# facebookresearch/co-tracker

Measured on AMD Instinct MI355X. Metric: tracked-point-frames/sec (N*T/s), higher is better.
Workload: dtype f32 (Linear layers as split-half f16 MFMA x3, f32 accumulate); 1 GPU; 512x512 T=120 N=6400 cotracker3 online-weights sliding window S=16 (BASELINE.json configs[2]); points_per_gpu=6400, frames=120, iters=6, window_len=16, offline=False, precision=f16x3, weights=seeded synthetic (no checkpoints offline)

## Files before the change

### co-tracker_amd/csrc/attention.hip

```cpp
#include "ctk_common.h"
#include "ctk_options.h"
#include "ctk_profile.h"
#include "gemm_params.h"
#include <cstdlib>

namespace {

constexpr int HD = CTK_HEAD_DIM;
constexpr int KC = 16;
constexpr int MAXB = 8;
constexpr int BPAD = 4;
constexpr float NEG_MAX = -3.402823466e+38f;

struct AttnP {
  const float* q; long q_ld, q_bs, q_is;
  const float* k; const float* v; long kv_ld, kv_bs, kv_is;
  float* out; long o_ld, o_bs, o_is;
  int nbatch, n1, n2;
  int splits, keys_per_split;
  float* partial;
  int o_split;
  int bpw;
  int qtiles;
  float scale;
  float scale2;
  int log2m;
  const uint8_t* kmask;
  const uint8_t* qmask;
  int binner;
  long q_obs, kv_obs, o_obs;
  long km_obs, qm_obs;
};

__device__ __forceinline__ long batch_row(const int b, const int binner, const long bs, const long obs, int* bo_out = nullptr) {
  const int bo = b / binner;
  if (bo_out) *bo_out = bo;
  return (long)bo * obs + (long)(b - bo * binner) * bs;
}

__global__ __launch_bounds__(64) void attention_kernel(AttnP p) {
  extern __shared__ __attribute__((aligned(16))) float smem[];
  float* lk = smem;
  float* lv = smem + p.bpw * (KC * HD + BPAD);
  const int lane = threadIdx.x;
  const int head = blockIdx.y;
  const int split = blockIdx.z;

  int b0, bl, qi;
  if (p.n1 >= 64) {
    b0 = blockIdx.x / p.qtiles;
    bl = 0;
    qi = (blockIdx.x % p.qtiles) * 64 + lane;
  } else {
    b0 = blockIdx.x * p.bpw;
    bl = lane / p.n1;
    qi = lane % p.n1;
  }
  const int nb_here = min(p.bpw, p.nbatch - b0);
  const bool active = (bl < nb_here) && (qi < p.n1);
  const int myb = b0 + min(bl, nb_here - 1);
  const int myq = min(qi, p.n1 - 1);

  float qr[HD];
  {
    const float* qp = p.q + (batch_row(myb, p.binner, p.q_bs, p.q_obs) + myq * p.q_is) * p.q_ld + head * HD;
#pragma unroll
    for (int d = 0; d < HD; d += 4) {
      const f32x4 t = *reinterpret_cast<const f32x4*>(qp + d);
      qr[d] = t[0] * p.scale; qr[d + 1] = t[1] * p.scale; qr[d + 2] = t[2] * p.scale; qr[d + 3] = t[3] * p.scale;
    }
  }
  float acc[HD];
#pragma unroll
  for (int d = 0; d < HD; ++d) acc[d] = 0.0f;
  float m = -INFINITY, l = 0.0f;
  int mybo;
  const long myorow = batch_row(myb, p.binner, p.o_bs, p.o_obs, &mybo) + myq * p.o_is;
  const bool qmasked = p.qmask && !p.qmask[mybo * p.qm_obs + myq];
  const uint8_t* mykmask = p.kmask ? p.kmask + mybo * p.km_obs : nullptr;

  const int kbeg = split * p.keys_per_split;
  const int kend = min(p.n2, kbeg + p.keys_per_split);
  const int bstride = KC * HD + BPAD;
  const float* myk = lk + min(bl, nb_here - 1) * bstride;
  const float* myv = lv + min(bl, nb_here - 1) * bstride;

  for (int k0 = kbeg; k0 < kend; k0 += KC) {
    const int kn = min(KC, kend - k0);
    __syncthreads();
    const int items = nb_here * kn * (HD / 4);
    for (int i = lane; i < items; i += 64) {
      const int d4 = i % (HD / 4);
      const int kk = (i / (HD / 4)) % kn;
      const int bb = i / ((HD / 4) * kn);
      const long row = (batch_row(b0 + bb, p.binner, p.kv_bs, p.kv_obs) + (long)(k0 + kk) * p.kv_is) * p.kv_ld + head * HD + d4 * 4;
      *reinterpret_cast<f32x4*>(&lk[bb * bstride + kk * HD + d4 * 4]) = *reinterpret_cast<const f32x4*>(p.k + row);
      *reinterpret_cast<f32x4*>(&lv[bb * bstride + kk * HD + d4 * 4]) = *reinterpret_cast<const f32x4*>(p.v + row);
    }
    __syncthreads();

    float s[KC];
    float cmax = -INFINITY;
#pragma unroll
    for (int kk = 0; kk < KC; ++kk) {
      float dot = 0.0f;
      if (kk < kn) {
#pragma unroll
        for (int d = 0; d < HD; d += 4) {
          const f32x4 t = *reinterpret_cast<const f32x4*>(myk + kk * HD + d);
          dot += qr[d] * t[0] + qr[d + 1] * t[1] + qr[d + 2] * t[2] + qr[d + 3] * t[3];
        }
        if (mykmask && !mykmask[k0 + kk]) dot = NEG_MAX;
        if (qmasked) dot = NEG_MAX;
        cmax = fmaxf(cmax, dot);
      } else {
        dot = -INFINITY;
      }
      s[kk] = dot;
    }
    const float mnew = fmaxf(m, cmax);
    const float alpha = expf(m - mnew);
    l *= alpha;
#pragma unroll
    for (int d = 0; d < HD; ++d) acc[d] *= alpha;
#pragma unroll
    for (int kk = 0; kk < KC; ++kk) {
      if (kk < kn) {
        const float pr = expf(s[kk] - mnew);
        l += pr;
#pragma unroll
        for (int d = 0; d < HD; d += 4) {
          const f32x4 t = *reinterpret_cast<const f32x4*>(myv + kk * HD + d);
          acc[d] += pr * t[0]; acc[d + 1] += pr * t[1]; acc[d + 2] += pr * t[2]; acc[d + 3] += pr * t[3];
        }
      }
    }
    m = mnew;
  }

  if (!active) return;
  if (p.splits == 1) {
    const float inv = 1.0f / l;
    float* op = p.out + myorow * p.o_ld + head * HD;
    _Float16* oh = reinterpret_cast<_Float16*>(p.out) + myorow * p.o_ld;
#pragma unroll
    for (int d = 0; d < HD; d += 4) {
      f32x4 t = {acc[d] * inv, acc[d + 1] * inv, acc[d + 2] * inv, acc[d + 3] * inv};
      if (p.o_split) {
        f16x4 hi, lo;
        ctk_split4(t, hi, lo);
        _Float16* dst = oh + ctk_sh_col(head * HD + d);
        *reinterpret_cast<f16x4*>(dst) = hi;
        *reinterpret_cast<f16x4*>(dst + 32) = lo;
      } else {
        *reinterpret_cast<f32x4*>(op + d) = t;
      }
    }
  } else {
    float* pp = p.partial + ((((long)split * p.nbatch + myb) * CTK_HEADS + head) * p.n1 + myq) * (HD + 2);
    pp[0] = m;
    pp[1] = l;
#pragma unroll
    for (int d = 0; d < HD; ++d) pp[2 + d] = acc[d];
  }
}

constexpr int KP = 56;
constexpr int VP = 72;
constexpr float PSCALE = 4096.0f;
constexpr int QT_PER_WG = 4;

constexpr int VT_PITCH = 52;
constexpr int VT_BYTES = 32 * VT_PITCH * 4;
constexpr int OIMG_PITCH = 208;
constexpr int OIMG_BYTES = 32 * OIMG_PITCH;

__device__ __forceinline__ int oimg_pos(const bool odd_head, const int d0) {
  if (!odd_head) return d0 < 32 ? d0 * 2 : 128 + (d0 - 32) * 2;
  return d0 < 16 ? 128 + d0 * 2 : (d0 - 16) * 2;
}

template <class RowPtr>
__device__ __forceinline__ void attn_store_sh_head(const f32x16 (&oacc)[2], const float inv, unsigned char* img ,
                                                   const int lane, const int head, RowPtr row_ptr) {
  const int r32 = lane & 31, half = lane >> 5;
  const bool odd = head & 1;
  unsigned char* wr = img + r32 * OIMG_PITCH;
#pragma unroll
  for (int dt = 0; dt < 2; ++dt)
#pragma unroll
    for (int q = 0; q < 4; ++q) {
      if (dt == 1 && q >= 2) continue;
      const int d0 = dt * 32 + q * 8 + half * 4;
      const f32x4 t = {oacc[dt][4 * q] * inv, oacc[dt][4 * q + 1] * inv, oacc[dt][4 * q + 2] * inv, oacc[dt][4 * q + 3] * inv};
      f16x4 hi, lo;
      ctk_split4(t, hi, lo);
      const int pos = oimg_pos(odd, d0);
      *reinterpret_cast<f16x4*>(wr + pos) = hi;
      *reinterpret_cast<f16x4*>(wr + pos + (pos < 128 ? 64 : 32)) = lo;
    }
  const int line_full = odd ? (3 * head + 1) / 2 : (3 * head) / 2;
  const int line_part = odd ? (3 * head) / 2 : (3 * head) / 2 + 1;
  const int part_off = odd ? 32 : 0;
#pragma unroll
  for (int k = 0; k < 6; ++k) {
    const int idx = k * 64 + lane, row = idx / 12, c = idx - row * 12;
    const f16x8 v = *reinterpret_cast<const f16x8*>(img + row * OIMG_PITCH + c * 16);
    _Float16* base = row_ptr(row);
    const int off = c < 8 ? line_full * 128 + c * 16 : line_part * 128 + part_off + (c < 10 ? (c - 8) * 16 : 64 + (c - 10) * 16);
    if (base) *reinterpret_cast<f16x8*>(reinterpret_cast<unsigned char*>(base) + off) = v;
  }
}

__global__ __launch_bounds__(256) void attention_kv64_kernel(AttnP p) {
  __shared__ __attribute__((aligned(16))) _Float16 lds[2 * 64 * KP + 2 * 64 * VP + 4 * OIMG_BYTES / 2];
  _Float16* kimg = lds;
  _Float16* vimg = lds + 2 * 64 * KP;
  const int tid = threadIdx.x, wave = tid >> 6, lane = tid & 63, r32 = lane & 31, half = lane >> 5;
  const int head = blockIdx.y, b = blockIdx.z;
  unsigned char* oimg = reinterpret_cast<unsigned char*>(lds + 2 * 64 * KP + 2 * 64 * VP) + wave * OIMG_BYTES;
  int bo;
  const long kvb = batch_row(b, p.binner, p.kv_bs, p.kv_obs, &bo);
  const long qb = batch_row(b, p.binner, p.q_bs, p.q_obs), ob = batch_row(b, p.binner, p.o_bs, p.o_obs);
  const uint8_t* kmask = p.kmask ? p.kmask + bo * p.km_obs : nullptr;
  const uint8_t* qmask = p.qmask ? p.qmask + bo * p.qm_obs : nullptr;

  for (int i = tid; i < 64 * (HD / 4); i += 256) {
    const int key = i / (HD / 4), d4 = i - key * (HD / 4);
    const long row = (kvb + (long)key * p.kv_is) * p.kv_ld + head * HD + d4 * 4;
    const f32x4 kk = *reinterpret_cast<const f32x4*>(p.k + row);
    const f32x4 vv = *reinterpret_cast<const f32x4*>(p.v + row);
    f16x4 hi, lo;
    ctk_split4(kk, hi, lo);
    *reinterpret_cast<f16x4*>(kimg + key * KP + d4 * 4) = hi;
    *reinterpret_cast<f16x4*>(kimg + 64 * KP + key * KP + d4 * 4) = lo;
    ctk_split4(vv, hi, lo);
    const int ko = key & 15;
    const int pos = (key & ~15) + 8 * ((ko >> 2) & 1) + 4 * (ko >> 3) + (ko & 3);
#pragma unroll
    for (int e = 0; e < 4; ++e) {
      vimg[(d4 * 4 + e) * VP + pos] = hi[e];
      vimg[64 * VP + (d4 * 4 + e) * VP + pos] = lo[e];
    }
  }

  f32x4 qraw[6];
  auto load_q = [&](int q0) {
    const int qi = min(q0 + r32, p.n1 - 1);
    const float* qp = p.q + (qb + (long)qi * p.q_is) * p.q_ld + head * HD + half * 8;
#pragma unroll
    for (int j = 0; j < 3; ++j) {
      qraw[2 * j] = *reinterpret_cast<const f32x4*>(qp + 16 * j);
      qraw[2 * j + 1] = *reinterpret_cast<const f32x4*>(qp + 16 * j + 4);
    }
  };
  const int q_first = blockIdx.x * QT_PER_WG * 128 + wave * 32;
  if (q_first < p.n1) load_q(q_first);
  __syncthreads();

  for (int qt = 0; qt < QT_PER_WG; ++qt) {
    const int q0 = q_first + qt * 128;
    if (q0 >= p.n1) break;
    const int qi = min(q0 + r32, p.n1 - 1);
    f16x8 qh[3], ql[3];
#pragma unroll
    for (int j = 0; j < 3; ++j) ctk_split8(qraw[2 * j] * p.scale2, qraw[2 * j + 1] * p.scale2, qh[j], ql[j]);
    if (qt + 1 < QT_PER_WG && q0 + 128 < p.n1) load_q(q0 + 128);
    f32x16 sacc[2];
#pragma unroll
    for (int kt = 0; kt < 2; ++kt) {
#pragma unroll
      for (int e = 0; e < 16; ++e) sacc[kt][e] = 0.0f;
#pragma unroll
      for (int j = 0; j < 3; ++j) {
        const _Float16* ka = kimg + (kt * 32 + r32) * KP + j * 16 + half * 8;
        const f16x8 kh = *reinterpret_cast<const f16x8*>(ka);
        const f16x8 kl = *reinterpret_cast<const f16x8*>(ka + 64 * KP);
        sacc[kt] = ctk_mma3(kh, kl, qh[j], ql[j], sacc[kt]);
      }
    }
    if (kmask || qmask) {
      const bool qm = qmask && !qmask[qi];
#pragma unroll
      for (int kt = 0; kt < 2; ++kt)
#pragma unroll
        for (int e = 0; e < 16; ++e) {
          const int key = 32 * kt + 8 * (e >> 2) + 4 * half + (e & 3);
          if (qm || (kmask && !kmask[key])) sacc[kt][e] = NEG_MAX;
        }
    }
    float mx = -INFINITY;
#pragma unroll
    for (int kt = 0; kt < 2; ++kt)
#pragma unroll
      for (int e = 0; e < 16; ++e) mx = fmaxf(mx, sacc[kt][e]);
    mx = fmaxf(mx, __shfl_xor(mx, 32, 64));
    float sum = 0.0f;
#pragma unroll
    for (int kt = 0; kt < 2; ++kt)
#pragma unroll
      for (int e = 0; e < 16; ++e) {
        const float pv = __builtin_amdgcn_exp2f(sacc[kt][e] - mx);
        sum += pv;
        sacc[kt][e] = pv * PSCALE;
      }
    sum += __shfl_xor(sum, 32, 64);
    f32x16 oacc[2];
#pragma unroll
    for (int dt = 0; dt < 2; ++dt)
#pragma unroll
      for (int e = 0; e < 16; ++e) oacc[dt][e] = 0.0f;
#pragma unroll
    for (int s = 0; s < 4; ++s) {
      const int kt = s >> 1, base = 8 * (s & 1);
      const f32x4 a = {sacc[kt][base], sacc[kt][base + 1], sacc[kt][base + 2], sacc[kt][base + 3]};
      const f32x4 c = {sacc[kt][base + 4], sacc[kt][base + 5], sacc[kt][base + 6], sacc[kt][base + 7]};
      f16x8 ph, pl;
      ctk_split8(a, c, ph, pl);
#pragma unroll
      for (int dt = 0; dt < 2; ++dt) {
        const _Float16* va = vimg + (dt * 32 + r32) * VP + s * 16 + half * 8;
        const f16x8 vh = *reinterpret_cast<const f16x8*>(va);
        const f16x8 vl = *reinterpret_cast<const f16x8*>(va + 64 * VP);
        oacc[dt] = ctk_mma3(vh, vl, ph, pl, oacc[dt]);
      }
    }
    const float inv = 1.0f / (sum * PSCALE);
    if (p.o_split) {
      attn_store_sh_head(oacc, inv, oimg, lane, head, [&](int row) -> _Float16* {
        const int qr = q0 + row;
        return qr < p.n1 ? reinterpret_cast<_Float16*>(p.out) + (ob + (long)qr * p.o_is) * p.o_ld : nullptr;
      });
    } else if (q0 + r32 < p.n1) {
      const long orow = (ob + (long)qi * p.o_is) * p.o_ld;
#pragma unroll
      for (int dt = 0; dt < 2; ++dt)
#pragma unroll
        for (int q = 0; q < 4; ++q) {
          const int d = dt * 32 + q * 8 + half * 4;
          if (d < HD) {
            const f32x4 t = {oacc[dt][4 * q] * inv, oacc[dt][4 * q + 1] * inv, oacc[dt][4 * q + 2] * inv, oacc[dt][4 * q + 3] * inv};
            *reinterpret_cast<f32x4*>(p.out + orow + head * HD + d) = t;
          }
        }
    }
  }
}

__global__ __launch_bounds__(256) void attention_q64_kernel(AttnP p) {
  __shared__ __attribute__((aligned(16))) float red[4][64][HD + 2];
  static_assert(VT_BYTES <= (int)sizeof(float) * 64 * (HD + 2), "the V transpose image fits a wave's slice of red");
  static_assert((VT_PITCH * 4) % 16 == 0 && (64 * (HD + 2) * 4) % 16 == 0, "16-byte rows / slices for ds_write_b128");
  const int tid = threadIdx.x, wave = tid >> 6, lane = tid & 63, r32 = lane & 31, half = lane >> 5;
  const int split = blockIdx.x, head = blockIdx.y, b = blockIdx.z;
  int bo;
  const long kvb = batch_row(b, p.binner, p.kv_bs, p.kv_obs, &bo);
  const long qb = batch_row(b, p.binner, p.q_bs, p.q_obs), ob = batch_row(b, p.binner, p.o_bs, p.o_obs);
  const uint8_t* kmask = p.kmask ? p.kmask + bo * p.km_obs : nullptr;
  const uint8_t* qmask = p.qmask ? p.qmask + bo * p.qm_obs : nullptr;

  f16x8 qh[2][3], ql[2][3];
#pragma unroll
  for (int qt = 0; qt < 2; ++qt) {
    const float* qp = p.q + (qb + (long)(qt * 32 + r32) * p.q_is) * p.q_ld + head * HD + half * 8;
#pragma unroll
    for (int j = 0; j < 3; ++j) {
      const f32x4 a = *reinterpret_cast<const f32x4*>(qp + 16 * j) * p.scale2;
      const f32x4 c = *reinterpret_cast<const f32x4*>(qp + 16 * j + 4) * p.scale2;
      ctk_split8(a, c, qh[qt][j], ql[qt][j]);
    }
  }
  const int kbeg = split * p.keys_per_split;
  const int kend = min(p.n2, kbeg + p.keys_per_split);
  const int ntiles = (kend - kbeg + 31) >> 5;
  const float* kbase = p.k + kvb * p.kv_ld + head * HD + half * 8;
  const float* vbase = p.v + kvb * p.kv_ld + head * HD;
  const long kstride = p.kv_is * p.kv_ld;
  const int vd0 = r32, vd1 = min(32 + r32, HD - 1);

  f32x4 kraw[6], vrow[6];
  float* vt = &red[wave][0][0];
  auto load_tile = [&](int tile) {
    const int k0 = kbeg + tile * 32;
    const long row = (long)min(k0 + r32, kend - 1) * kstride;
    const float* kp = kbase + row;
    const float* vp = vbase + row + half * 8;
#pragma unroll
    for (int j = 0; j < 3; ++j) {
      kraw[2 * j] = *reinterpret_cast<const f32x4*>(kp + 16 * j);
      kraw[2 * j + 1] = *reinterpret_cast<const f32x4*>(kp + 16 * j + 4);
      vrow[2 * j] = *reinterpret_cast<const f32x4*>(vp + 16 * j);
      vrow[2 * j + 1] = *reinterpret_cast<const f32x4*>(vp + 16 * j + 4);
    }
  };

  float m[2] = {-INFINITY, -INFINITY}, l[2] = {0.0f, 0.0f};
  f32x16 oacc[2][2];
#pragma unroll
  for (int dt = 0; dt < 2; ++dt)
#pragma unroll
    for (int qt = 0; qt < 2; ++qt)
#pragma unroll
      for (int e = 0; e < 16; ++e) oacc[dt][qt][e] = 0.0f;

  if (wave < ntiles) load_tile(wave);
  for (int tile = wave; tile < ntiles; tile += 4) {
    const int k0 = kbeg + tile * 32;
    f16x8 kh[3], kl[3], vh[2][2], vl[2][2];
#pragma unroll
    for (int j = 0; j < 3; ++j) ctk_split8(kraw[2 * j], kraw[2 * j + 1], kh[j], kl[j]);
    {
      float* wrow = vt + r32 * VT_PITCH + half * 8;
#pragma unroll
      for (int j = 0; j < 3; ++j) {
        *reinterpret_cast<f32x4*>(wrow + 16 * j) = vrow[2 * j];
        *reinterpret_cast<f32x4*>(wrow + 16 * j + 4) = vrow[2 * j + 1];
      }
      __builtin_amdgcn_wave_barrier();
      float vraw[2][16];
#pragma unroll
      for (int s = 0; s < 2; ++s)
#pragma unroll
        for (int e = 0; e < 8; ++e) {
          const int key = 16 * s + 8 * (e >> 2) + 4 * half + (e & 3);
          vraw[0][s * 8 + e] = vt[key * VT_PITCH + vd0];
          vraw[1][s * 8 + e] = vt[key * VT_PITCH + vd1];
        }
      __builtin_amdgcn_wave_barrier();
#pragma unroll
      for (int dt = 0; dt < 2; ++dt)
#pragma unroll
        for (int s = 0; s < 2; ++s) {
          const f32x4 a = {vraw[dt][s * 8], vraw[dt][s * 8 + 1], vraw[dt][s * 8 + 2], vraw[dt][s * 8 + 3]};
          const f32x4 c = {vraw[dt][s * 8 + 4], vraw[dt][s * 8 + 5], vraw[dt][s * 8 + 6], vraw[dt][s * 8 + 7]};
          ctk_split8(a, c, vh[dt][s], vl[dt][s]);
        }
    }
    if (tile + 4 < ntiles) load_tile(tile + 4);

    f32x16 sacc[2];
#pragma unroll
    for (int qt = 0; qt < 2; ++qt) {
#pragma unroll
      for (int e = 0; e < 16; ++e) sacc[qt][e] = 0.0f;
#pragma unroll
      for (int j = 0; j < 3; ++j) sacc[qt] = ctk_mma3(kh[j], kl[j], qh[qt][j], ql[qt][j], sacc[qt]);
    }
    if (kmask || qmask) {
#pragma unroll
      for (int e = 0; e < 16; ++e) {
        const int key = min(k0 + 8 * (e >> 2) + 4 * half + (e & 3), kend - 1);
        const bool km = kmask && !kmask[key];
#pragma unroll
        for (int qt = 0; qt < 2; ++qt)
          if (km || (qmask && !qmask[qt * 32 + r32])) sacc[qt][e] = NEG_MAX;
      }
    }
    if (k0 + 32 > kend) {
#pragma unroll
      for (int e = 0; e < 16; ++e) {
        const int key = k0 + 8 * (e >> 2) + 4 * half + (e & 3);
        if (key >= kend) {
          sacc[0][e] = -INFINITY;
          sacc[1][e] = -INFINITY;
        }
      }
    }
    f16x8 ph[2][2], pl[2][2];
#pragma unroll
    for (int qt = 0; qt < 2; ++qt) {
      float tmax = -INFINITY;
#pragma unroll
      for (int e = 0; e < 16; ++e) tmax = fmaxf(tmax, sacc[qt][e]);
      tmax = fmaxf(tmax, __shfl_xor(tmax, 32, 64));
      const float mnew = fmaxf(m[qt], tmax);
      const float alpha = __builtin_amdgcn_exp2f(m[qt] - mnew);
      m[qt] = mnew;
      float psum = 0.0f;
#pragma unroll
      for (int e = 0; e < 16; ++e) {
        const float pv = __builtin_amdgcn_exp2f(sacc[qt][e] - mnew);
        psum += pv;
        sacc[qt][e] = pv * PSCALE;
      }
      l[qt] = l[qt] * alpha + psum;
#pragma unroll
      for (int e = 0; e < 16; ++e) {
        oacc[0][qt][e] *= alpha;
        oacc[1][qt][e] *= alpha;
      }
#pragma unroll
      for (int s = 0; s < 2; ++s) {
        const f32x4 a = {sacc[qt][8 * s], sacc[qt][8 * s + 1], sacc[qt][8 * s + 2], sacc[qt][8 * s + 3]};
        const f32x4 c = {sacc[qt][8 * s + 4], sacc[qt][8 * s + 5], sacc[qt][8 * s + 6], sacc[qt][8 * s + 7]};
        ctk_split8(a, c, ph[qt][s], pl[qt][s]);
      }
    }
#pragma unroll
    for (int s = 0; s < 2; ++s)
#pragma unroll
      for (int dt = 0; dt < 2; ++dt)
#pragma unroll
        for (int qt = 0; qt < 2; ++qt) oacc[dt][qt] = ctk_mma3(vh[dt][s], vl[dt][s], ph[qt][s], pl[qt][s], oacc[dt][qt]);
  }

#pragma unroll
  for (int qt = 0; qt < 2; ++qt) {
    const float lsum = l[qt] + __shfl_xor(l[qt], 32, 64);
    float* rr = &red[wave][qt * 32 + r32][0];
    if (half == 0) {
      rr[0] = m[qt];
      rr[1] = lsum;
    }
#pragma unroll
    for (int dt = 0; dt < 2; ++dt)
#pragma unroll
      for (int q = 0; q < 4; ++q) {
        const int d = dt * 32 + q * 8 + half * 4;
        if (d < HD) {
#pragma unroll
          for (int e = 0; e < 4; ++e) rr[2 + d + e] = oacc[dt][qt][4 * q + e] * (1.0f / PSCALE);
        }
      }
  }
  __syncthreads();
  {
    const int qi = tid >> 2, part = tid & 3;
    float mm = -INFINITY;
#pragma unroll
    for (int w = 0; w < 4; ++w) mm = fmaxf(mm, red[w][qi][0]);
    float L = 0.0f, o[12];
#pragma unroll
    for (int d = 0; d < 12; ++d) o[d] = 0.0f;
#pragma unroll
    for (int w = 0; w < 4; ++w) {
      const float wm = red[w][qi][0];
      const float wgt = (wm == -INFINITY) ? 0.0f : __builtin_amdgcn_exp2f(wm - mm);
      L += wgt * red[w][qi][1];
#pragma unroll
      for (int d = 0; d < 12; ++d) o[d] += wgt * red[w][qi][2 + part * 12 + d];
    }
    if (p.splits == 1) {
      const float inv = 1.0f / L;
      const long orow = (ob + (long)qi * p.o_is) * p.o_ld;
#pragma unroll
      for (int i = 0; i < 3; ++i) {
        const f32x4 t = {o[4 * i] * inv, o[4 * i + 1] * inv, o[4 * i + 2] * inv, o[4 * i + 3] * inv};
        const int col = head * HD + part * 12 + 4 * i;
        if (p.o_split) {
          f16x4 hi, lo;
          ctk_split4(t, hi, lo);
          _Float16* dst = reinterpret_cast<_Float16*>(p.out) + orow + ctk_sh_col(col);
          *reinterpret_cast<f16x4*>(dst) = hi;
          *reinterpret_cast<f16x4*>(dst + 32) = lo;
        } else {
          *reinterpret_cast<f32x4*>(p.out + orow + col) = t;
        }
      }
    } else {
      float* pp = p.partial + ((((long)split * p.nbatch + b) * CTK_HEADS + head) * p.n1 + qi) * (HD + 2);
      if (part == 0) {
        pp[0] = mm;
        pp[1] = L;
      }
#pragma unroll
      for (int d = 0; d < 12; ++d) pp[2 + part * 12 + d] = o[d];
    }
  }
}

template <int PACK>
__global__ __launch_bounds__(256, 2) void attention_self_kernel(AttnP p) {
  __shared__ __attribute__((aligned(16))) unsigned char oimg_all[4 * OIMG_BYTES];
  const int wave = threadIdx.x >> 6, lane = threadIdx.x & 63, r32 = lane & 31, half = lane >> 5;
  unsigned char* oimg = oimg_all + wave * OIMG_BYTES;
  const int head = blockIdx.y;
  constexpr int pack = PACK;
  constexpr int spb = 32 / pack;
  const long job = (long)blockIdx.x * 4 + wave;
  const long njobs = (long)((p.nbatch + pack - 1) / pack) * p.qtiles;
  if (job >= njobs) return;
  const int g = (int)(job / p.qtiles), qtile = (int)(job - (long)g * p.qtiles);
  const int b0 = g * pack;

  const int qb = r32 / spb, qi = qtile * spb + r32 % spb;
  const bool qvalid = (b0 + qb < p.nbatch) && (qi < p.n1);
  const int qbc = min(b0 + qb, p.nbatch - 1), qic = min(qi, p.n1 - 1);
  f16x8 qh[3], ql[3];
  {
    const float* qp = p.q + ((long)qbc * p.q_bs + (long)qic * p.q_is) * p.q_ld + head * HD + half * 8;
#pragma unroll
    for (int j = 0; j < 3; ++j) {
      const f32x4 a = *reinterpret_cast<const f32x4*>(qp + 16 * j) * p.scale2;
      const f32x4 c = *reinterpret_cast<const f32x4*>(qp + 16 * j + 4) * p.scale2;
      ctk_split8(a, c, qh[j], ql[j]);
    }
  }
  const int vd0 = r32, vd1 = min(32 + r32, HD - 1);
  float m = -INFINITY, l = 0.0f;
  f32x16 oacc[2];
#pragma unroll
  for (int dt = 0; dt < 2; ++dt)
#pragma unroll
    for (int e = 0; e < 16; ++e) oacc[dt][e] = 0.0f;

  const int nkt = (pack == 2) ? 1 : (p.n2 + 31) / 32;
  for (int kt = 0; kt < nkt; ++kt) {
    f16x8 kh[3], kl[3], vh[2][2], vl[2][2];
    {
      const int kb = min(b0 + r32 / spb, p.nbatch - 1), ki = min(kt * spb + r32 % spb, p.n2 - 1);
      const float* kp = p.k + ((long)kb * p.kv_bs + (long)ki * p.kv_is) * p.kv_ld + head * HD + half * 8;
#pragma unroll
      for (int j = 0; j < 3; ++j)
        ctk_split8(*reinterpret_cast<const f32x4*>(kp + 16 * j), *reinterpret_cast<const f32x4*>(kp + 16 * j + 4), kh[j], kl[j]);
    }
#pragma unroll
    for (int s = 0; s < 2; ++s) {
      float v0[8], v1[8];
#pragma unroll
      for (int e = 0; e < 8; ++e) {
        const int slot = 16 * s + 8 * (e >> 2) + 4 * half + (e & 3);
        const int kb = min(b0 + slot / spb, p.nbatch - 1), ki = min(kt * spb + slot % spb, p.n2 - 1);
        const float* vp = p.v + ((long)kb * p.kv_bs + (long)ki * p.kv_is) * p.kv_ld + head * HD;
        v0[e] = vp[vd0];
        v1[e] = vp[vd1];
      }
      ctk_split8(f32x4{v0[0], v0[1], v0[2], v0[3]}, f32x4{v0[4], v0[5], v0[6], v0[7]}, vh[0][s], vl[0][s]);
      ctk_split8(f32x4{v1[0], v1[1], v1[2], v1[3]}, f32x4{v1[4], v1[5], v1[6], v1[7]}, vh[1][s], vl[1][s]);
    }
    f32x16 sacc;
#pragma unroll
    for (int e = 0; e < 16; ++e) sacc[e] = 0.0f;
#pragma unroll
    for (int j = 0; j < 3; ++j) sacc = ctk_mma3(kh[j], kl[j], qh[j], ql[j], sacc);
    float tmax = -INFINITY;
#pragma unroll
    for (int e = 0; e < 16; ++e) {
      const int slot = 8 * (e >> 2) + 4 * half + (e & 3);
      const bool ok = (slot / spb == qb) && (b0 + slot / spb < p.nbatch) && (kt * spb + slot % spb < p.n2);
      if (ok && ((p.kmask && !p.kmask[min(kt * spb + slot % spb, p.n2 - 1)]) || (p.qmask && !p.qmask[qic]))) sacc[e] = NEG_MAX;
      sacc[e] = ok ? sacc[e] : -INFINITY;
      tmax = fmaxf(tmax, sacc[e]);
    }
    tmax = fmaxf(tmax, __shfl_xor(tmax, 32, 64));
    float mnew = fmaxf(m, tmax);
    if (mnew == -INFINITY) mnew = 0.0f;
    const float alpha = __builtin_amdgcn_exp2f(m - mnew);
    m = mnew;
    float psum = 0.0f;
#pragma unroll
    for (int e = 0; e < 16; ++e) {
      const float pv = __builtin_amdgcn_exp2f(sacc[e] - mnew);
      psum += pv;
      sacc[e] = pv * PSCALE;
    }
    l = l * alpha + psum;
#pragma unroll
    for (int e = 0; e < 16; ++e) {
      oacc[0][e] *= alpha;
      oacc[1][e] *= alpha;
    }
#pragma unroll
    for (int s = 0; s < 2; ++s) {
      f16x8 ph, pl;
      ctk_split8(f32x4{sacc[8 * s], sacc[8 * s + 1], sacc[8 * s + 2], sacc[8 * s + 3]},
                 f32x4{sacc[8 * s + 4], sacc[8 * s + 5], sacc[8 * s + 6], sacc[8 * s + 7]}, ph, pl);
      oacc[0] = ctk_mma3(vh[0][s], vl[0][s], ph, pl, oacc[0]);
      oacc[1] = ctk_mma3(vh[1][s], vl[1][s], ph, pl, oacc[1]);
    }
  }
  l += __shfl_xor(l, 32, 64);
  const float inv = 1.0f / (l * PSCALE);
  if (p.o_split) {
    attn_store_sh_head(oacc, inv, oimg, lane, head, [&](int row) -> _Float16* {
      const int ob = b0 + row / spb, oi = qtile * spb + row % spb;
      return (ob < p.nbatch && oi < p.n1) ? reinterpret_cast<_Float16*>(p.out) + ((long)ob * p.o_bs + (long)oi * p.o_is) * p.o_ld : nullptr;
    });
  } else if (qvalid) {
    const long orow = ((long)qbc * p.o_bs + (long)qic * p.o_is) * p.o_ld;
#pragma unroll
    for (int dt = 0; dt < 2; ++dt)
#pragma unroll
      for (int q = 0; q < 4; ++q) {
        const int d = dt * 32 + q * 8 + half * 4;
        if (d < HD) {
          const f32x4 t = {oacc[dt][4 * q] * inv, oacc[dt][4 * q + 1] * inv, oacc[dt][4 * q + 2] * inv, oacc[dt][4 * q + 3] * inv};
          *reinterpret_cast<f32x4*>(p.out + orow + head * HD + d) = t;
        }
      }
  }
}

struct TimeRaw {
  f32x4 q[6], k[6], v[6];
};

__global__ __launch_bounds__(256, 2) void attention_time16_kernel(AttnP p, long njobs) {
  __shared__ __attribute__((aligned(16))) unsigned char oimg_all[4 * (OIMG_BYTES + VT_BYTES)];
  const int wave = threadIdx.x >> 6, lane = threadIdx.x & 63, r32 = lane & 31, half = lane >> 5;
  unsigned char* oimg = oimg_all + wave * (OIMG_BYTES + VT_BYTES);
  float* vt = reinterpret_cast<float*>(oimg + OIMG_BYTES);
  const long stride = (long)gridDim.x * 4;
  long job = (long)blockIdx.x * 4 + wave;
  if (job >= njobs) return;
  const int vd0 = r32, vd1 = min(32 + r32, HD - 1);
  const int rb = r32 >> 4, ri = r32 & 15;

  auto slot_of = [&](const int i, const int ln) { return ((64 * i + ln) * 43691) >> 19; };
  auto chunk_of = [&](const int i, const int ln) { return (64 * i + ln) - 12 * slot_of(i, ln); };
  auto load = [&](long jb, TimeRaw& r) {
    int ln = lane;
    asm volatile("" : "+v"(ln));
    const int head = (int)(jb % CTK_HEADS);
    const int b0 = (int)(jb / CTK_HEADS) * 2;
    const float* qb = p.q + head * HD;
    const float* kb = p.k + head * HD;
    const float* vb = p.v + head * HD;
#pragma unroll
    for (int i = 0; i < 6; ++i) {
      const int row = slot_of(i, ln), c = chunk_of(i, ln);
      const int bc = min(b0 + (row >> 4), p.nbatch - 1), fr = row & 15;
      const long qo = ((long)bc * p.q_bs + (long)min(fr, p.n1 - 1) * p.q_is) * p.q_ld + c * 4;
      const long ko = ((long)bc * p.kv_bs + (long)min(fr, p.n2 - 1) * p.kv_is) * p.kv_ld + c * 4;
      r.q[i] = *reinterpret_cast<const f32x4*>(qb + qo);
      r.k[i] = *reinterpret_cast<const f32x4*>(kb + ko);
      r.v[i] = *reinterpret_cast<const f32x4*>(vb + ko);
      __builtin_amdgcn_sched_barrier(0);
    }
  };
  auto stage = [&](const f32x4 (&m)[6]) {
    int ln = lane;
    asm volatile("" : "+v"(ln));
#pragma unroll
    for (int i = 0; i < 6; ++i) *reinterpret_cast<f32x4*>(vt + slot_of(i, ln) * VT_PITCH + chunk_of(i, ln) * 4) = m[i];
    __builtin_amdgcn_wave_barrier();
  };
  auto frag_rows = [&](f32x4 (&f)[6]) {
    const float* rr = vt + r32 * VT_PITCH + half * 8;
#pragma unroll
    for (int j = 0; j < 3; ++j) {
      f[2 * j] = *reinterpret_cast<const f32x4*>(rr + 16 * j);
      f[2 * j + 1] = *reinterpret_cast<const f32x4*>(rr + 16 * j + 4);
    }
    __builtin_amdgcn_wave_barrier();
  };

  TimeRaw raw;
  load(job, raw);
  while (true) {
    const int head = (int)(job % CTK_HEADS);
    const int b0 = (int)(job / CTK_HEADS) * 2;
    f16x8 qh[3], ql[3], kh[3], kl[3], vh[2][2], vl[2][2];
    {
      f32x4 f[6];
      stage(raw.q);
      frag_rows(f);
#pragma unroll
      for (int j = 0; j < 3; ++j) ctk_split8(f[2 * j] * p.scale2, f[2 * j + 1] * p.scale2, qh[j], ql[j]);
      stage(raw.k);
      frag_rows(f);
#pragma unroll
      for (int j = 0; j < 3; ++j) ctk_split8(f[2 * j], f[2 * j + 1], kh[j], kl[j]);
    }
    {
      stage(raw.v);
      float v0[16], v1[16];
#pragma unroll
      for (int s = 0; s < 2; ++s)
#pragma unroll
        for (int e = 0; e < 8; ++e) {
          const int slot = 16 * s + 8 * (e >> 2) + 4 * half + (e & 3);
          v0[8 * s + e] = vt[slot * VT_PITCH + vd0];
          v1[8 * s + e] = vt[slot * VT_PITCH + vd1];
        }
      __builtin_amdgcn_wave_barrier();
#pragma unroll
      for (int s = 0; s < 2; ++s) {
        ctk_split8(f32x4{v0[8 * s], v0[8 * s + 1], v0[8 * s + 2], v0[8 * s + 3]}, f32x4{v0[8 * s + 4], v0[8 * s + 5], v0[8 * s + 6], v0[8 * s + 7]},
                   vh[0][s], vl[0][s]);
        ctk_split8(f32x4{v1[8 * s], v1[8 * s + 1], v1[8 * s + 2], v1[8 * s + 3]}, f32x4{v1[8 * s + 4], v1[8 * s + 5], v1[8 * s + 6], v1[8 * s + 7]},
                   vh[1][s], vl[1][s]);
      }
    }
    const long next = job + stride;
    const bool more = next < njobs;
    if (more) load(next, raw);

    const bool qvalid = (b0 + rb < p.nbatch) && (ri < p.n1);
    f32x16 sacc;
#pragma unroll
    for (int e = 0; e < 16; ++e) sacc[e] = 0.0f;
#pragma unroll
    for (int j = 0; j < 3; ++j) sacc = ctk_mma3(kh[j], kl[j], qh[j], ql[j], sacc);
    float tmax = -INFINITY;
#pragma unroll
    for (int e = 0; e < 16; ++e) {
      const int slot = 8 * (e >> 2) + 4 * half + (e & 3);
      const bool ok = ((slot >> 4) == rb) && (b0 + (slot >> 4) < p.nbatch) && ((slot & 15) < p.n2);
      sacc[e] = ok ? sacc[e] : -INFINITY;
      tmax = fmaxf(tmax, sacc[e]);
    }
    tmax = fmaxf(tmax, __shfl_xor(tmax, 32, 64));
    const float mnew = (tmax == -INFINITY) ? 0.0f : tmax;
    float l = 0.0f;
#pragma unroll
    for (int e = 0; e < 16; ++e) {
      const float pv = __builtin_amdgcn_exp2f(sacc[e] - mnew);
      l += pv;
      sacc[e] = pv * PSCALE;
    }
    f32x16 oacc[2];
#pragma unroll
    for (int dt = 0; dt < 2; ++dt)
#pragma unroll
      for (int e = 0; e < 16; ++e) oacc[dt][e] = 0.0f;
#pragma unroll
    for (int s = 0; s < 2; ++s) {
      f16x8 ph, pl;
      ctk_split8(f32x4{sacc[8 * s], sacc[8 * s + 1], sacc[8 * s + 2], sacc[8 * s + 3]},
                 f32x4{sacc[8 * s + 4], sacc[8 * s + 5], sacc[8 * s + 6], sacc[8 * s + 7]}, ph, pl);
      oacc[0] = ctk_mma3(vh[0][s], vl[0][s], ph, pl, oacc[0]);
      oacc[1] = ctk_mma3(vh[1][s], vl[1][s], ph, pl, oacc[1]);
    }
    l += __shfl_xor(l, 32, 64);
    const float inv = 1.0f / (l * PSCALE);
    if (p.o_split) {
      attn_store_sh_head(oacc, inv, oimg, lane, head, [&](int row) -> _Float16* {
        const int ob = b0 + (row >> 4), oi = row & 15;
        return (ob < p.nbatch && oi < p.n1) ? reinterpret_cast<_Float16*>(p.out) + ((long)ob * p.o_bs + (long)oi * p.o_is) * p.o_ld : nullptr;
      });
    } else if (qvalid) {
      const long orow = ((long)(b0 + rb) * p.o_bs + (long)ri * p.o_is) * p.o_ld;
#pragma unroll
      for (int dt = 0; dt < 2; ++dt)
#pragma unroll
        for (int q = 0; q < 4; ++q) {
          const int d = dt * 32 + q * 8 + half * 4;
          if (d < HD) {
            const f32x4 t = {oacc[dt][4 * q] * inv, oacc[dt][4 * q + 1] * inv, oacc[dt][4 * q + 2] * inv, oacc[dt][4 * q + 3] * inv};
            *reinterpret_cast<f32x4*>(p.out + orow + head * HD + d) = t;
          }
        }
    }
    if (!more) break;
    job = next;
  }
}

__global__ void attention_merge_kernel(AttnP p) {
  const long i = (long)blockIdx.x * blockDim.x + threadIdx.x;
  const long total = (long)p.nbatch * CTK_HEADS * p.n1 * HD;
  if (i >= total) return;
  const int d = i % HD;
  long r = i / HD;
  const int qi = r % p.n1; r /= p.n1;
  const int head = r % CTK_HEADS;
  const int b = r / CTK_HEADS;
  const long stride = (long)p.nbatch * CTK_HEADS * p.n1 * (HD + 2);
  const float* base = p.partial + (((long)b * CTK_HEADS + head) * p.n1 + qi) * (HD + 2);
  float m = -INFINITY;
  for (int s = 0; s < p.splits; ++s) m = fmaxf(m, base[s * stride]);
  float l = 0.0f, a = 0.0f;
  for (int s = 0; s < p.splits; ++s) {
    const float w = p.log2m ? __builtin_amdgcn_exp2f(base[s * stride] - m) : expf(base[s * stride] - m);
    l += w * base[s * stride + 1];
    a += w * base[s * stride + 2 + d];
  }
  const float o = a / l;
  const long orow = batch_row(b, p.binner, p.o_bs, p.o_obs) + qi * p.o_is;
  if (p.o_split) {
    _Float16* oh = reinterpret_cast<_Float16*>(p.out) + orow * p.o_ld + ctk_sh_col(head * HD + d);
    const _Float16 hi = (_Float16)o;
    oh[0] = hi;
    oh[32] = (_Float16)(o - (float)hi);
  } else {
    p.out[orow * p.o_ld + head * HD + d] = o;
  }
}

int attn_backend() { return ctk_opt(CTK_OPT_ATTENTION_VALU); }

}

extern "C" int ctk_attention(const ctk_attn_args* a, void* stream) { return ctk_attention_ex(a, nullptr, stream); }

extern "C" int ctk_attention_ex(const ctk_attn_args* a, const ctk_attn_batch2* b2, void* stream) {
  if (!a || !a->q || !a->k || !a->v || !a->out) return CTK_E_NULL;
  if (a->nbatch <= 0 || a->n1 <= 0 || a->n2 <= 0) return CTK_E_SHAPE;
  const bool two_level = b2 != nullptr && b2->inner > 0;
  if (two_level && (a->nbatch % b2->inner)) return CTK_E_SHAPE;
  if ((a->q_ld % 4) || (a->kv_ld % 4) || (a->o_ld % 4)) return CTK_E_ALIGN;
  if (!ctk_aligned16(a->q) || !ctk_aligned16(a->k) || !ctk_aligned16(a->v) || !ctk_aligned16(a->out)) return CTK_E_ALIGN;
  AttnP p;
  p.q = a->q; p.q_ld = a->q_ld; p.q_bs = a->q_bs; p.q_is = a->q_is;
  p.k = a->k; p.v = a->v; p.kv_ld = a->kv_ld; p.kv_bs = a->kv_bs; p.kv_is = a->kv_is;
  p.out = static_cast<float*>(a->out); p.o_ld = a->o_ld; p.o_bs = a->o_bs; p.o_is = a->o_is;
  p.o_split = a->o_split;
  if (p.o_split && (a->o_ld % 64)) return CTK_E_ALIGN;
  p.nbatch = a->nbatch; p.n1 = a->n1; p.n2 = a->n2;
  p.splits = a->splits > 1 ? a->splits : 1;
  if (p.splits > 1 && !a->partial) return CTK_E_NULL;
  p.partial = a->partial;
  p.kmask = a->key_mask;
  p.qmask = a->query_mask;
  p.binner = two_level ? b2->inner : a->nbatch;
  p.q_obs = two_level ? b2->q_os : 0; p.kv_obs = two_level ? b2->kv_os : 0; p.o_obs = two_level ? b2->o_os : 0;
  p.km_obs = two_level ? b2->key_mask_os : 0; p.qm_obs = two_level ? b2->query_mask_os : 0;
  p.scale = 0.14433756729740643f;
  p.scale2 = 0.14433756729740643f * 1.4426950408889634f;
  p.log2m = 0;
  hipStream_t s = static_cast<hipStream_t>(stream);
  const double flops = 4.0 * a->nbatch * (double)a->n1 * a->n2 * CTK_HID;
  const double bytes = 4.0 * a->nbatch * ((double)a->n1 * 2 + (double)a->n2 * 2) * CTK_HID;
  const bool mfma = attn_backend() == 0;

  if (mfma && a->n2 == CTK_VIRT) {
    p.splits = 1;
    p.keys_per_split = a->n2;
    p.bpw = 1;
    p.qtiles = 1;
    CtkProfScope ps(a->n1 > CTK_VIRT ? "attention_p2v" : "attention_vself", flops, bytes, s);
    const unsigned gx = (unsigned)((a->n1 + 128 * QT_PER_WG - 1) / (128 * QT_PER_WG));
    hipLaunchKernelGGL(attention_kv64_kernel, dim3(gx, CTK_HEADS, (unsigned)a->nbatch), dim3(256), 0, s, p);
    CTK_HIP_CHECK_LAUNCH();
    return CTK_OK;
  }
  if (mfma && a->n1 == CTK_VIRT && a->n2 > CTK_VIRT) {
    p.keys_per_split = ((a->n2 + p.splits - 1) / p.splits + 31) / 32 * 32;
    p.splits = (a->n2 + p.keys_per_split - 1) / p.keys_per_split;
    p.bpw = 1;
    p.qtiles = 1;
    p.log2m = 1;
    CtkProfScope ps("attention_v2p", flops, bytes, s);
    hipLaunchKernelGGL(attention_q64_kernel, dim3((unsigned)p.splits, CTK_HEADS, (unsigned)a->nbatch), dim3(256), 0, s, p);
    CTK_HIP_CHECK_LAUNCH();
    if (p.splits > 1) {
      const long total = (long)p.nbatch * CTK_HEADS * p.n1 * HD;
      hipLaunchKernelGGL(attention_merge_kernel, dim3((unsigned)((total + 255) / 256)), dim3(256), 0, s, p);
      CTK_HIP_CHECK_LAUNCH();
    }
    return CTK_OK;
  }

  if (mfma && a->n1 == a->n2 && p.splits == 1 && !two_level) {
    p.keys_per_split = a->n2;
    p.bpw = a->n1 <= 16 ? 2 : 1;
    p.qtiles = p.bpw == 2 ? 1 : (a->n1 + 31) / 32;
    const long njobs = (long)((a->nbatch + p.bpw - 1) / p.bpw) * p.qtiles;
    CtkProfScope ps(a->q_is == 1 ? "attention_time" : "attention_vself", flops, bytes, s);
    const bool persistent = ctk_opt(CTK_OPT_ATTENTION_TIME_PERSISTENT) != 0;
    if (p.bpw == 2 && !p.kmask && !p.qmask && persistent) {
      const long total = njobs * CTK_HEADS;
      const unsigned blocks = (unsigned)((total + 3) / 4 < 512 ? (total + 3) / 4 : 512);
      hipLaunchKernelGGL(attention_time16_kernel, dim3(blocks), dim3(256), 0, s, p, total);
    } else if (p.bpw == 2) hipLaunchKernelGGL(attention_self_kernel<2>, dim3((unsigned)((njobs + 3) / 4), CTK_HEADS), dim3(256), 0, s, p);
    else hipLaunchKernelGGL(attention_self_kernel<1>, dim3((unsigned)((njobs + 3) / 4), CTK_HEADS), dim3(256), 0, s, p);
    CTK_HIP_CHECK_LAUNCH();
    return CTK_OK;
  }

  p.keys_per_split = ((a->n2 + p.splits - 1) / p.splits + KC - 1) / KC * KC;
  p.splits = (a->n2 + p.keys_per_split - 1) / p.keys_per_split;
  unsigned gx;
  if (a->n1 >= 64) {
    p.bpw = 1;
    p.qtiles = (a->n1 + 63) / 64;
    gx = (unsigned)(p.qtiles * a->nbatch);
  } else {
    p.bpw = 64 / a->n1;
    if (p.bpw > MAXB) p.bpw = MAXB;
    p.qtiles = 1;
    gx = (unsigned)((a->nbatch + p.bpw - 1) / p.bpw);
  }
  const char* pname = p.splits > 1 ? "attention_v2p" : (a->n1 > CTK_VIRT && a->n2 == CTK_VIRT) ? "attention_p2v"
                      : (a->n1 == CTK_VIRT && a->n2 == CTK_VIRT && a->q_is != 1) ? "attention_vself" : "attention_time";
  CtkProfScope ps(pname, flops, bytes, s);
  const size_t lds_bytes = (size_t)2 * p.bpw * (KC * HD + BPAD) * sizeof(float);
  hipLaunchKernelGGL(attention_kernel, dim3(gx, CTK_HEADS, (unsigned)p.splits), dim3(64), lds_bytes, s, p);
  CTK_HIP_CHECK_LAUNCH();
  if (p.splits > 1) {
    const long total = (long)p.nbatch * CTK_HEADS * p.n1 * HD;
    hipLaunchKernelGGL(attention_merge_kernel, dim3((unsigned)((total + 255) / 256)), dim3(256), 0, s, p);
    CTK_HIP_CHECK_LAUNCH();
  }
  return CTK_OK;
}
```

Measured before the change: 650,100 tracked-point-frames/s.

## Stage split-f16 K/V tiles cooperatively in LDS for q64 attention

The virtual-to-point attention kernel now runs 512 threads, with each wave owning one 32-query tile and one of four key slots. Groups of 128 keys are loaded cooperatively, split into hi/lo f16 once, and written to double-buffered LDS images, with V stored pre-transposed into MFMA fragment order. This removes the redundant per-wave V transpose and repeated splitting, and overlaps the next group's global loads with compute. In exchange it adds a block-wide barrier per group and a larger LDS footprint, which may lower occupancy.

```diff
diff --git a/co-tracker_amd/csrc/attention.hip b/co-tracker_amd/csrc/attention.hip
--- a/co-tracker_amd/csrc/attention.hip
+++ b/co-tracker_amd/csrc/attention.hip
@@ -347,11 +347,19 @@
   }
 }
 
-__global__ __launch_bounds__(256) void attention_q64_kernel(AttnP p) {
-  __shared__ __attribute__((aligned(16))) float red[4][64][HD + 2];
-  static_assert(VT_BYTES <= (int)sizeof(float) * 64 * (HD + 2), "the V transpose image fits a wave's slice of red");
-  static_assert((VT_PITCH * 4) % 16 == 0 && (64 * (HD + 2) * 4) % 16 == 0, "16-byte rows / slices for ds_write_b128");
-  const int tid = threadIdx.x, wave = tid >> 6, lane = tid & 63, r32 = lane & 31, half = lane >> 5;
+constexpr int Q64_KP = 56;
+constexpr int Q64_VP = 136;
+constexpr int Q64_KIMG = 128 * Q64_KP;
+constexpr int Q64_VIMG = HD * Q64_VP;
+constexpr int Q64_BUF = 2 * Q64_KIMG + 2 * Q64_VIMG;
+
+__global__ __launch_bounds__(512) void attention_q64_kernel(AttnP p) {
+  __shared__ __attribute__((aligned(16))) _Float16 stage[2 * Q64_BUF];
+  float (*red)[64][HD + 2] = reinterpret_cast<float (*)[64][HD + 2]>(stage);
+  static_assert(sizeof(float) * 4 * 64 * (HD + 2) <= sizeof(_Float16) * Q64_BUF, "the four slot states fit one fragment image");
+  static_assert((Q64_KP * 2) % 16 == 0 && (Q64_VP * 2) % 16 == 0 && (Q64_KIMG * 2) % 16 == 0 && (Q64_VIMG * 2) % 16 == 0, "16-byte rows / planes for ds_read_b128");
+  const int tid = threadIdx.x, hw = tid >> 6, lane = tid & 63, r32 = lane & 31, half = lane >> 5;
+  const int slot = hw & 3, qt = hw >> 2;
   const int split = blockIdx.x, head = blockIdx.y, b = blockIdx.z;
   int bo;
   const long kvb = batch_row(b, p.binner, p.kv_bs, p.kv_obs, &bo);
@@ -359,157 +367,163 @@
   const uint8_t* kmask = p.kmask ? p.kmask + bo * p.km_obs : nullptr;
   const uint8_t* qmask = p.qmask ? p.qmask + bo * p.qm_obs : nullptr;
 
-  f16x8 qh[2][3], ql[2][3];
-#pragma unroll
-  for (int qt = 0; qt < 2; ++qt) {
+  f16x8 qh[3], ql[3];
+  {
     const float* qp = p.q + (qb + (long)(qt * 32 + r32) * p.q_is) * p.q_ld + head * HD + half * 8;
 #pragma unroll
     for (int j = 0; j < 3; ++j) {
       const f32x4 a = *reinterpret_cast<const f32x4*>(qp + 16 * j) * p.scale2;
       const f32x4 c = *reinterpret_cast<const f32x4*>(qp + 16 * j + 4) * p.scale2;
-      ctk_split8(a, c, qh[qt][j], ql[qt][j]);
+      ctk_split8(a, c, qh[j], ql[j]);
     }
   }
   const int kbeg = split * p.keys_per_split;
   const int kend = min(p.n2, kbeg + p.keys_per_split);
   const int ntiles = (kend - kbeg + 31) >> 5;
-  const float* kbase = p.k + kvb * p.kv_ld + head * HD + half * 8;
+  const int ngroups = (ntiles + 3) >> 2;
+  const float* kbase = p.k + kvb * p.kv_ld + head * HD;
   const float* vbase = p.v + kvb * p.kv_ld + head * HD;
   const long kstride = p.kv_is * p.kv_ld;
   const int vd0 = r32, vd1 = min(32 + r32, HD - 1);
 
-  f32x4 kraw[6], vrow[6];
-  float* vt = &red[wave][0][0];
-  auto load_tile = [&](int tile) {
-    const int k0 = kbeg + tile * 32;
-    const long row = (long)min(k0 + r32, kend - 1) * kstride;
-    const float* kp = kbase + row;
-    const float* vp = vbase + row + half * 8;
-#pragma unroll
-    for (int j = 0; j < 3; ++j) {
-      kraw[2 * j] = *reinterpret_cast<const f32x4*>(kp + 16 * j);
-      kraw[2 * j + 1] = *reinterpret_cast<const f32x4*>(kp + 16 * j + 4);
-      vrow[2 * j] = *reinterpret_cast<const f32x4*>(vp + 16 * j);
-      vrow[2 * j + 1] = *reinterpret_cast<const f32x4*>(vp + 16 * j + 4);
+  f32x4 kraw[3], vraw[4];
+  const bool vloader = tid < 384;
+  const int vR = tid / 12, vc = tid - 12 * vR;
+  auto prefetch = [&](const int g) {
+    const int key0 = kbeg + g * 128;
+#pragma unroll
+    for (int i = 0; i < 3; ++i) {
+      const int idx = 512 * i + tid, row = idx / 12, c = idx - 12 * row;
+      kraw[i] = *reinterpret_cast<const f32x4*>(kbase + (long)min(key0 + row, kend - 1) * kstride + 4 * c);
+    }
+    if (vloader) {
+#pragma unroll
+      for (int i = 0; i < 4; ++i)
+        vraw[i] = *reinterpret_cast<const f32x4*>(vbase + (long)min(key0 + 4 * vR + i, kend - 1) * kstride + 4 * vc);
     }
   };
-
-  float m[2] = {-INFINITY, -INFINITY}, l[2] = {0.0f, 0.0f};
-  f32x16 oacc[2][2];
+  auto stage_group = [&](_Float16* buf) {
+    _Float16* kimg = buf;
+    _Float16* vimg = buf + 2 * Q64_KIMG;
+#pragma unroll
+    for (int i = 0; i < 3; ++i) {
+      const int idx = 512 * i + tid, row = idx / 12, c = idx - 12 * row;
+      f16x4 hi, lo;
+      ctk_split4(kraw[i], hi, lo);
+      *reinterpret_cast<f16x4*>(kimg + row * Q64_KP + 4 * c) = hi;
+      *reinterpret_cast<f16x4*>(kimg + Q64_KIMG + row * Q64_KP + 4 * c) = lo;
+    }
+    if (vloader) {
+      f16x4 hi[4], lo[4];
+#pragma unroll
+      for (int i = 0; i < 4; ++i) ctk_split4(vraw[i], hi[i], lo[i]);
+      const int kk = 4 * vR, ko = kk & 15;
+      const int pos = (kk & ~15) + 8 * ((ko >> 2) & 1) + 4 * (ko >> 3);
+#pragma unroll
+      for (int e = 0; e < 4; ++e) {
+        const f16x4 th = {hi[0][e], hi[1][e], hi[2][e], hi[3][e]};
+        const f16x4 tl = {lo[0][e], lo[1][e], lo[2][e], lo[3][e]};
+        *reinterpret_cast<f16x4*>(vimg + (4 * vc + e) * Q64_VP + pos) = th;
+        *reinterpret_cast<f16x4*>(vimg + Q64_VIMG + (4 * vc + e) * Q64_VP + pos) = tl;
+      }
+    }
+  };
+
+  float m = -INFINITY, l = 0.0f;
+  f32x16 oacc[2];
 #pragma unroll
   for (int dt = 0; dt < 2; ++dt)
 #pragma unroll
-    for (int qt = 0; qt < 2; ++qt)
-#pragma unroll
-      for (int e = 0; e < 16; ++e) oacc[dt][qt][e] = 0.0f;
-
-  if (wave < ntiles) load_tile(wave);
-  for (int tile = wave; tile < ntiles; tile += 4) {
+    for (int e = 0; e < 16; ++e) oacc[dt][e] = 0.0f;
+
+  prefetch(0);
+  for (int g = 0; g < ngroups; ++g) {
+    _Float16* buf = stage + (g & 1) * Q64_BUF;
+    stage_group(buf);
+    if (g + 1 < ngroups) prefetch(g + 1);
+    __syncthreads();
+    const int tile = 4 * g + slot;
+    if (tile >= ntiles) continue;
     const int k0 = kbeg + tile * 32;
     f16x8 kh[3], kl[3], vh[2][2], vl[2][2];
-#pragma unroll
-    for (int j = 0; j < 3; ++j) ctk_split8(kraw[2 * j], kraw[2 * j + 1], kh[j], kl[j]);
     {
-      float* wrow = vt + r32 * VT_PITCH + half * 8;
+      const _Float16* ka = buf + (slot * 32 + r32) * Q64_KP + half * 8;
 #pragma unroll
       for (int j = 0; j < 3; ++j) {
-        *reinterpret_cast<f32x4*>(wrow + 16 * j) = vrow[2 * j];
-        *reinterpret_cast<f32x4*>(wrow + 16 * j + 4) = vrow[2 * j + 1];
-      }
-      __builtin_amdgcn_wave_barrier();
-      float vraw[2][16];
-#pragma unroll
-      for (int s = 0; s < 2; ++s)
-#pragma unroll
-        for (int e = 0; e < 8; ++e) {
-          const int key = 16 * s + 8 * (e >> 2) + 4 * half + (e & 3);
-          vraw[0][s * 8 + e] = vt[key * VT_PITCH + vd0];
-          vraw[1][s * 8 + e] = vt[key * VT_PITCH + vd1];
-        }
-      __builtin_amdgcn_wave_barrier();
-#pragma unroll
-      for (int dt = 0; dt < 2; ++dt)
-#pragma unroll
-        for (int s = 0; s < 2; ++s) {
-          const f32x4 a = {vraw[dt][s * 8], vraw[dt][s * 8 + 1], vraw[dt][s * 8 + 2], vraw[dt][s * 8 + 3]};
-          const f32x4 c = {vraw[dt][s * 8 + 4], vraw[dt][s * 8 + 5], vraw[dt][s * 8 + 6], vraw[dt][s * 8 + 7]};
-          ctk_split8(a, c, vh[dt][s], vl[dt][s]);
-        }
-    }
-    if (tile + 4 < ntiles) load_tile(tile + 4);
-
-    f32x16 sacc[2];
-#pragma unroll
-    for (int qt = 0; qt < 2; ++qt) {
-#pragma unroll
-      for (int e = 0; e < 16; ++e) sacc[qt][e] = 0.0f;
-#pragma unroll
-      for (int j = 0; j < 3; ++j) sacc[qt] = ctk_mma3(kh[j], kl[j], qh[qt][j], ql[qt][j], sacc[qt]);
-    }
+        kh[j] = *reinterpret_cast<const f16x8*>(ka + 16 * j);
+        kl[j] = *reinterpret_cast<const f16x8*>(ka + Q64_KIMG + 16 * j);
+      }
+      const _Float16* va = buf + 2 * Q64_KIMG + slot * 32 + half * 8;
+#pragma unroll
+      for (int s = 0; s < 2; ++s) {
+        vh[0][s] = *reinterpret_cast<const f16x8*>(va + vd0 * Q64_VP + 16 * s);
+        vl[0][s] = *reinterpret_cast<const f16x8*>(va + Q64_VIMG + vd0 * Q64_VP + 16 * s);
+        vh[1][s] = *reinterpret_cast<const f16x8*>(va + vd1 * Q64_VP + 16 * s);
+        vl[1][s] = *reinterpret_cast<const f16x8*>(va + Q64_VIMG + vd1 * Q64_VP + 16 * s);
+      }
+    }
+
+    f32x16 sacc;
+#pragma unroll
+    for (int e = 0; e < 16; ++e) sacc[e] = 0.0f;
+#pragma unroll
+    for (int j = 0; j < 3; ++j) sacc = ctk_mma3(kh[j], kl[j], qh[j], ql[j], sacc);
     if (kmask || qmask) {
 #pragma unroll
       for (int e = 0; e < 16; ++e) {
         const int key = min(k0 + 8 * (e >> 2) + 4 * half + (e & 3), kend - 1);
         const bool km = kmask && !kmask[key];
-#pragma unroll
-        for (int qt = 0; qt < 2; ++qt)
-          if (km || (qmask && !qmask[qt * 32 + r32])) sacc[qt][e] = NEG_MAX;
+        if (km || (qmask && !qmask[qt * 32 + r32])) sacc[e] = NEG_MAX;
       }
     }
     if (k0 + 32 > kend) {
 #pragma unroll
       for (int e = 0; e < 16; ++e) {
         const int key = k0 + 8 * (e >> 2) + 4 * half + (e & 3);
-        if (key >= kend) {
-          sacc[0][e] = -INFINITY;
-          sacc[1][e] = -INFINITY;
-        }
-      }
-    }
-    f16x8 ph[2][2], pl[2][2];
-#pragma unroll
-    for (int qt = 0; qt < 2; ++qt) {
+        if (key >= kend) sacc[e] = -INFINITY;
+      }
+    }
+    f16x8 ph[2], pl[2];
+    {
       float tmax = -INFINITY;
 #pragma unroll
-      for (int e = 0; e < 16; ++e) tmax = fmaxf(tmax, sacc[qt][e]);
+      for (int e = 0; e < 16; ++e) tmax = fmaxf(tmax, sacc[e]);
       tmax = fmaxf(tmax, __shfl_xor(tmax, 32, 64));
-      const float mnew = fmaxf(m[qt], tmax);
-      const float alpha = __builtin_amdgcn_exp2f(m[qt] - mnew);
-      m[qt] = mnew;
+      const float mnew = fmaxf(m, tmax);
+      const float alpha = __builtin_amdgcn_exp2f(m - mnew);
+      m = mnew;
       float psum = 0.0f;
 #pragma unroll
       for (int e = 0; e < 16; ++e) {
-        const float pv = __builtin_amdgcn_exp2f(sacc[qt][e] - mnew);
+        const float pv = __builtin_amdgcn_exp2f(sacc[e] - mnew);
         psum += pv;
-        sacc[qt][e] = pv * PSCALE;
-      }
-      l[qt] = l[qt] * alpha + psum;
+        sacc[e] = pv * PSCALE;
+      }
+      l = l * alpha + psum;
 #pragma unroll
       for (int e = 0; e < 16; ++e) {
-        oacc[0][qt][e] *= alpha;
-        oacc[1][qt][e] *= alpha;
+        oacc[0][e] *= alpha;
+        oacc[1][e] *= alpha;
       }
 #pragma unroll
       for (int s = 0; s < 2; ++s) {
-        const f32x4 a = {sacc[qt][8 * s], sacc[qt][8 * s + 1], sacc[qt][8 * s + 2], sacc[qt][8 * s + 3]};
-        const f32x4 c = {sacc[qt][8 * s + 4], sacc[qt][8 * s + 5], sacc[qt][8 * s + 6], sacc[qt][8 * s + 7]};
-        ctk_split8(a, c, ph[qt][s], pl[qt][s]);
+        const f32x4 a = {sacc[8 * s], sacc[8 * s + 1], sacc[8 * s + 2], sacc[8 * s + 3]};
+        const f32x4 c = {sacc[8 * s + 4], sacc[8 * s + 5], sacc[8 * s + 6], sacc[8 * s + 7]};
+        ctk_split8(a, c, ph[s], pl[s]);
       }
     }
 #pragma unroll
     for (int s = 0; s < 2; ++s)
 #pragma unroll
-      for (int dt = 0; dt < 2; ++dt)
-#pragma unroll
-        for (int qt = 0; qt < 2; ++qt) oacc[dt][qt] = ctk_mma3(vh[dt][s], vl[dt][s], ph[qt][s], pl[qt][s], oacc[dt][qt]);
-  }
-
-#pragma unroll
-  for (int qt = 0; qt < 2; ++qt) {
-    const float lsum = l[qt] + __shfl_xor(l[qt], 32, 64);
-    float* rr = &red[wave][qt * 32 + r32][0];
+      for (int dt = 0; dt < 2; ++dt) oacc[dt] = ctk_mma3(vh[dt][s], vl[dt][s], ph[s], pl[s], oacc[dt]);
+  }
+
+  __syncthreads();
+  {
+    const float lsum = l + __shfl_xor(l, 32, 64);
+    float* rr = &red[slot][qt * 32 + r32][0];
     if (half == 0) {
-      rr[0] = m[qt];
+      rr[0] = m;
       rr[1] = lsum;
     }
 #pragma unroll
@@ -519,12 +533,12 @@
         const int d = dt * 32 + q * 8 + half * 4;
         if (d < HD) {
 #pragma unroll
-          for (int e = 0; e < 4; ++e) rr[2 + d + e] = oacc[dt][qt][4 * q + e] * (1.0f / PSCALE);
+          for (int e = 0; e < 4; ++e) rr[2 + d + e] = oacc[dt][4 * q + e] * (1.0f / PSCALE);
         }
       }
   }
   __syncthreads();
-  {
+  if (tid < 256) {
     const int qi = tid >> 2, part = tid & 3;
     float mm = -INFINITY;
 #pragma unroll
@@ -932,7 +946,7 @@
     p.qtiles = 1;
     p.log2m = 1;
     CtkProfScope ps("attention_v2p", flops, bytes, s);
-    hipLaunchKernelGGL(attention_q64_kernel, dim3((unsigned)p.splits, CTK_HEADS, (unsigned)a->nbatch), dim3(256), 0, s, p);
+    hipLaunchKernelGGL(attention_q64_kernel, dim3((unsigned)p.splits, CTK_HEADS, (unsigned)a->nbatch), dim3(512), 0, s, p);
     CTK_HIP_CHECK_LAUNCH();
     if (p.splits > 1) {
       const long total = (long)p.nbatch * CTK_HEADS * p.n1 * HD;
```

Result: no change. 651,700 tracked-point-frames/s, median of 6 (+0.2%).
